# Manta-Network/manta-rs

Measured on AMD Instinct MI355X. Metric: G1 MSM Mscalar/s at 2^20, higher is better.
Workload: dtype u32; 1 GPU; 2^20 BLS12-381 G1 variable-base MSM per GPU, uniform scalars resident in HBM; curve=BLS12-381, log_n=20, window_bits=17, msms_in_flight=3

## Files before the change

manta_rs_amd/csrc/msm_accumulate.h:

```cpp
#pragma once
#include "msm_common.h"

namespace mg {

#ifdef MG_ACC_WAVES
#define MG_ACC_ATTR __attribute__((amdgpu_waves_per_eu(MG_ACC_WAVES, MG_ACC_WAVES)))
#else
#define MG_ACC_ATTR
#endif
template <class F, bool PROBE = false>
__global__ __launch_bounds__(256) MG_ACC_ATTR void accumulate_chunks(const u32 *__restrict__ keys, const u32 *__restrict__ vals,
                                                         u32 M, u32 L, u32 invalid, const u32 *__restrict__ bases,
                                                         u32 astride, u32 *__restrict__ buckets,
                                                         u32 *__restrict__ pkeys, u32 *__restrict__ ppts, u32 T,
                                                         const u32 *__restrict__ count, unsigned long long *__restrict__ clk,
                                                         u32 adapt) {
    const u32 t = blockIdx.x * blockDim.x + threadIdx.x;
    if (t >= T) return;
    long long c0 = 0;
    unsigned long long w0 = 0;
    if constexpr (PROBE)
        if (t == 0) c0 = clock64(), w0 = wall_clock64();
    if (count) {
        M = *count;
        if (adapt) {
            const u32 l = (M + T - 1) / T;
            L = l > L ? l : L;
        }
    }
    const size_t begin = (size_t)t * L;
    size_t end = begin + L;
    if (end > M) end = M;
    u32 cur = begin < M ? keys[begin] : invalid;
    if (cur == invalid) {
        pkeys[2 * t] = invalid;
        pkeys[2 * t + 1] = invalid;
        return;
    }
    XYZZ<F> acc = XYZZ<F>::inf();
    bool first = true;
    for (size_t j = begin; j < end; ++j) {
        const u32 k = keys[j];
        if (k != cur) {
            if (first) {
                pkeys[2 * t] = cur;
                acc.store(ppts + (size_t)(2 * t) * XYZZ<F>::WORDS);
                first = false;
            } else {
                acc.store(buckets + (size_t)cur * XYZZ<F>::WORDS);
            }
            acc = XYZZ<F>::inf();
            cur = k;
            if (k == invalid) break;
        }
        const u32 v = vals[j];
        const Affine<F> p = Affine<F>::load(bases + (size_t)(v & 0x7fffffffu) * astride);
        acc.madd_throughput(p, (v >> 31) != 0);
    }
    if (first) {
        pkeys[2 * t] = cur;
        acc.store(ppts + (size_t)(2 * t) * XYZZ<F>::WORDS);
        pkeys[2 * t + 1] = cur;
        XYZZ<F>::inf().store(ppts + (size_t)(2 * t + 1) * XYZZ<F>::WORDS);
    } else {
        pkeys[2 * t + 1] = cur;
        acc.store(ppts + (size_t)(2 * t + 1) * XYZZ<F>::WORDS);
    }
    if constexpr (PROBE)
        if (t == 0) clk[0] = (unsigned long long)(clock64() - c0), clk[1] = wall_clock64() - w0;
}

template <class F> struct AccSingle {
    static constexpr int XW = XYZZ<F>::WORDS;
    static constexpr int PAIR = F::EXT ? 1 : 0;
    static constexpr int SLOTS = 256 >> PAIR, PER = SLOTS / 64;
    typedef CoopAdd<F, false> Coop;
    static constexpr size_t LDS_BYTES = ((size_t)SLOTS * XW + Coop::LDS_WORDS) * 4;
};
template <class F>
__global__ __launch_bounds__(256) MG_TAIL_ATTR void accumulate_single(const u32 *__restrict__ vals, u32 M, u32 L, const u32 *__restrict__ bases,
                                                                      u32 astride, u32 *__restrict__ pkeys, u32 *__restrict__ ppts, u32 T,
                                                                      const u32 *__restrict__ count, u32 adapt, u32 invalid) {
    extern __shared__ __attribute__((aligned(16))) u32 acc_single_lds[];
    constexpr int XW = AccSingle<F>::XW, PAIR = AccSingle<F>::PAIR, SLOTS = AccSingle<F>::SLOTS, PER = AccSingle<F>::PER;
    u32 *xs = acc_single_lds;
    u32 *cx = acc_single_lds + SLOTS * XW;
    const u32 t = blockIdx.x * blockDim.x + threadIdx.x;
    const int lane = threadIdx.x & 63, wave = threadIdx.x >> 6;
    if (count) {
        M = *count;
        if (adapt) {
            const u32 l = (M + T - 1) / T;
            L = l > L ? l : L;
        }
    }
    XYZZ<F> acc = XYZZ<F>::inf();
    const size_t begin = (size_t)t * L;
    size_t end = begin + L;
    if (end > M) end = M;
    if (t < T)
        for (size_t j = begin; j < end; ++j) {
            const u32 v = vals[j];
            const Affine<F> p = Affine<F>::load(bases + (size_t)(v & 0x7fffffffu) * astride);
            acc.madd_throughput(p, (v >> 31) != 0);
        }
    if ((size_t)blockIdx.x * blockDim.x * L >= M) {
        if (threadIdx.x == 0) pkeys[blockIdx.x] = invalid;
        return;
    }
    if constexpr (PAIR) acc.add(XYZZ<F>::shfl(acc, lane ^ 1));
    if (!PAIR || !(lane & 1)) acc.store(xs + (size_t)(threadIdx.x >> PAIR) * XW);
    __syncthreads();
    acc = XYZZ<F>::load(xs + (size_t)(lane * PER) * XW);
#pragma unroll 1
    for (int k = 1; k < PER; ++k) AccSingle<F>::Coop::add(acc, XYZZ<F>::load(xs + (size_t)(lane * PER + k) * XW), cx, wave, lane);
#pragma unroll 1
    for (int d = 1; d < 64; d <<= 1) AccSingle<F>::Coop::add(acc, XYZZ<F>::shfl(acc, lane ^ d), cx, wave, lane);
    if (threadIdx.x == 0) {
        pkeys[blockIdx.x] = 0u;
        acc.store(ppts + (size_t)blockIdx.x * XW);
    }
}

#ifdef MG_CALIBRATION
template <class F>
__global__ __launch_bounds__(256) void gather_only_chunks(const u32 *__restrict__ keys, const u32 *__restrict__ vals,
                                                          u32 M, u32 L, u32 invalid, const u32 *__restrict__ bases,
                                                          u32 astride, u32 *__restrict__ pkeys, u32 T,
                                                          const u32 *__restrict__ count) {
    const u32 t = blockIdx.x * blockDim.x + threadIdx.x;
    if (t >= T) return;
    if (count) M = *count;
    const size_t begin = (size_t)t * L;
    size_t end = begin + L;
    if (end > M) end = M;
    u32 x = 0;
    for (size_t j = begin; j < end; ++j) {
        const u32 k = keys[j];
        if (k == invalid) break;
        const u32 v = vals[j];
        const uint4 *p = reinterpret_cast<const uint4 *>(bases + (size_t)(v & 0x7fffffffu) * astride);
#pragma unroll
        for (int q = 0; q < (int)(Affine<F>::WORDS + 3) / 4; ++q) {
            const uint4 w = p[q];
            x ^= w.x ^ w.y ^ w.z ^ w.w;
        }
        x ^= k;
    }
    pkeys[2 * t] = invalid;
    pkeys[2 * t + 1] = invalid;
    if (x == 0x9e3779b9u) pkeys[2 * t] = invalid - 1;
}
#endif

}
```

manta_rs_amd/csrc/msm_engine.h:

```cpp
#pragma once
#include "msm_common.h"
#include "msm_digits.h"
#include "msm_accumulate.h"
#include "msm_reduce.h"
#include "msm_tables.h"

namespace mg {

template <class Curve, int GROUP> struct GT;
template <class Curve> struct GT<Curve, 1> {
#ifdef MG_G1_SATURATED
    typedef Fp<typename Curve::Fq> F;
#else
    typedef FpR<typename Curve::Fq> F;
#endif
    typedef Fp<typename Curve::Fq> FIO;
    typedef host::HFp<typename Curve::Fq> HF;
};
template <class Curve> struct GT<Curve, 2> {
#ifdef MG_G2_SATURATED
    typedef Fp2<typename Curve::Fq> F;
#else
    typedef Fp2R<typename Curve::Fq> F;
#endif
// ... 400 lines not shown
            if (hipEventElapsedTime(&ms, ws->t0, ws->t1) == hipSuccess) set_last_accumulate_ms(ms);
            const unsigned long long ck[2] = {((volatile unsigned long long *)ws->h_clk)[0], ((volatile unsigned long long *)ws->h_clk)[1]};
            int khz = 0, dev = 0;
            if (ck[1] && hipGetDevice(&dev) == hipSuccess &&
                hipDeviceGetAttribute(&khz, hipDeviceAttributeWallClockRate, dev) == hipSuccess)
                set_last_accumulate_mhz((float)((double)ck[0] / (double)ck[1] * (double)khz / 1e3));
        }
        const MsmPlan &pl = ws->plan;
        const MsmTail &t = ws->tail;
        const u32 Wb = (u32)pl.Wb, segs = t.segs, T1 = t.T1, nP = t.nP;
        const u32 *st = (const u32 *)ws->h_stage;
        for (u32 q = 0; q < ws->batch; ++q) {
        HP total = HP::inf();
        for (int w = (int)((q + 1) * Wb) - 1; w >= (int)(q * Wb); --w) {
            HP win;
            if (t.kind == TAIL_WINDOW_SUMS) {
                win = HP::from_xyzz_words(st + (size_t)w * XW_IO);
            } else if (t.kind == TAIL_X_SUMS) {
                const HP X = HP::from_xyzz_words(st + ((size_t)w * 2 + 0) * XW_IO);
                const HP sumS = HP::from_xyzz_words(st + ((size_t)w * 2 + 1) * XW_IO);
                win = HP::add(sumS, HP::mul_pow2(X, 6));
            } else {
                const u32 *A1 = st + ((size_t)w * T1) * XW_IO;
                const u32 *S1 = st + ((size_t)segs * T1 + (size_t)w * T1) * XW_IO;
                const u32 *P0 = st + ((size_t)segs * 2 * T1 + (size_t)w * nP) * XW_IO;
                HP sumS = HP::inf(), run = HP::inf(), uA = HP::inf();
                for (int u = (int)T1 - 1; u >= 0; --u) {
                    sumS = HP::add(sumS, HP::from_xyzz_words(S1 + (size_t)u * XW_IO));
                    if (u >= 1) {
                        run = HP::add(run, HP::from_xyzz_words(A1 + (size_t)u * XW_IO));
                        uA = HP::add(uA, run);
                    }
                }
                HP X = HP::add(sumS, HP::mul_pow2(uA, 6));
                HP sumP = HP::inf();
                for (u32 u = 0; u < nP; ++u) sumP = HP::add(sumP, HP::from_xyzz_words(P0 + (size_t)u * XW_IO));
                win = HP::add(sumP, HP::mul_pow2(X, 6));
            }
            if (t.tail_shift) win = HP::mul_pow2(win, t.tail_shift);
            for (u32 e = 0; e < t.n_extra; ++e) {
                const HP x = HP::from_xyzz_words(st + (t.extra_off_pts + (size_t)e * segs + (size_t)w) * XW_IO);
                win = HP::add(win, t.extra_shift[e] ? HP::mul_pow2(x, t.extra_shift[e]) : x);
            }
            if (w != (int)((q + 1) * Wb) - 1) total = HP::mul_pow2(total, (unsigned)pl.c);
            total = HP::add(total, win);
        }
        hp(out + q) = total;
        }
        return MG_OK;
    }

    int msm_fold_device(MsmWorkspace *ws, u32 *d_out, size_t out_stride_words, hipStream_t on = nullptr) override {
        if (!ws || !ws->pending || !d_out || !ws->tail.d_tail) return MG_ERR_STATE;
        const MsmTail &t = ws->tail;
        if (ws->plan.Wb != 1) return MG_ERR_STATE;
        FoldDesc d{t.d_tail, ws->extra.as<u32>(), t.kind, t.T1, t.nP, t.segs, t.n_extra, t.tail_shift, {}};
        for (u32 e = 0; e < t.n_extra; ++e) d.extra_shift[e] = t.extra_shift[e];
        hipLaunchKernelGGL((fold_windows<F>), dim3(ws->batch), dim3(64), 0, on ? on : msm_stream_of(ws), d, d_out, out_stride_words);
        MG_HIP(hipGetLastError());
        return MG_OK;
    }
    int msm_discard(MsmWorkspace *ws) override {
        if (!ws) return MG_ERR_STATE;
        ws->pending = 0;
        MG_HIP(hipStreamSynchronize(msm_stream_of(ws)));
        return MG_OK;
    }

    int fixed_base_mul(const u32 *base_affine_host, const u32 *d_scalars, size_t n, u32 *d_out_affine,
                       hipStream_t s) override {
        if (!s) s = setup_stream();
        u32 *d_base = nullptr, *tmp = nullptr;
        MG_HIP(hipMalloc((void **)&d_base, AW_IO * 4));
        hipError_t e = hipMalloc((void **)&tmp, n * XW_IO * 4);
        if (e != hipSuccess) {
            hipFree(d_base);
            set_last_hip_error(e, "hipMalloc(fixed_base tmp)", __FILE__, __LINE__);
            return MG_ERR_OOM;
        }
        hipMemcpyAsync(d_base, base_affine_host, AW_IO * 4, hipMemcpyHostToDevice, s);
        constexpr int KB = 16;
        u32 *t_xyzz = nullptr, *t_aff = nullptr;
        if (n >= msm_knobs().fixed_base_table_min) {
            constexpr size_t TN = 32 * 255;
            if (hipMalloc((void **)&t_xyzz, TN * XW_IO * 4) == hipSuccess && hipMalloc((void **)&t_aff, TN * AW_IO * 4) == hipSuccess) {
                hipLaunchKernelGGL((fixed_base_table_kernel<FIO>), dim3(cdiv(TN, 256)), dim3(256), 0, s, d_base, t_xyzz);
                hipLaunchKernelGGL((xyzz_to_affine_batch<FIO, KB>), dim3(cdiv(cdiv(TN, KB), 256)), dim3(256), 0, s, t_xyzz, TN, t_aff,
                                   (u32)AW_IO);
                hipLaunchKernelGGL((fixed_base_mul_table_kernel<FIO>), dim3(cdiv(n, 256)), dim3(256), 0, s, t_aff, d_scalars, n, tmp);
            } else {
                (void)hipGetLastError();
                if (t_xyzz) hipFree(t_xyzz);
                t_xyzz = nullptr;
            }
        }
        if (!t_xyzz)
        hipLaunchKernelGGL((fixed_base_mul_kernel<FIO>), dim3(cdiv(n, 256)), dim3(256), 0, s, d_base, d_scalars, n, tmp);
        hipLaunchKernelGGL((xyzz_to_affine_batch<FIO, KB>), dim3(cdiv(cdiv(n, KB), 256)), dim3(256), 0, s, tmp, n,
                           d_out_affine, (u32)AW_IO);
        e = hipStreamSynchronize(s);
        hipFree(d_base);
        hipFree(tmp);
        if (t_xyzz) hipFree(t_xyzz);
        if (t_aff) hipFree(t_aff);
        if (e != hipSuccess) {
            set_last_hip_error(e, "fixed_base_mul", __FILE__, __LINE__);
            return MG_ERR_HIP;
        }
        return MG_OK;
    }

    int ec_elementwise(int op, const u32 *a_host, const u32 *b_host, size_t n, u32 *out_affine_host) override {
        return ec_elementwise_impl(op, a_host, b_host, n, out_affine_host, false);
    }
    int ec_elementwise_xyzz(int op, const u32 *a_host, const u32 *b_host, size_t n, u32 *out_xyzz_host) override {
        return ec_elementwise_impl(op, a_host, b_host, n, out_xyzz_host, true);
    }
    int ec_mul_xyzz_begin(const u32 *a_host, const u32 *k_host, size_t n, MsmWorkspace *ws, const u32 *glv_beta_std) override {
        if (!a_host || !k_host || !n || !ws) return MG_ERR_ARG;
        const size_t ab = n * AW_IO * 4, bb = n * 32 + (glv_beta_std ? (size_t)AW_IO / 2 * 4 : 0), tb = n * XW_IO * 4;
        int rc = ws->scratch.reserve(ab + bb + tb);
        if (rc) return rc;
        unsigned char *d = (unsigned char *)ws->scratch.p;
        hipError_t e = hipMemcpyAsync(d, a_host, ab, hipMemcpyHostToDevice, ws->stream);
        if (e == hipSuccess) e = hipMemcpyAsync(d + ab, k_host, n * 32, hipMemcpyHostToDevice, ws->stream);
        if (e == hipSuccess && glv_beta_std)
            e = hipMemcpyAsync(d + ab + n * 32, glv_beta_std, (size_t)AW_IO / 2 * 4, hipMemcpyHostToDevice, ws->stream);
        if (e == hipSuccess) {
            hipLaunchKernelGGL((ec_elementwise_kernel<F>), dim3(cdiv(n, 256)), dim3(256), 0, ws->stream, glv_beta_std ? 6 : 3, (const u32 *)d,
                               (const u32 *)(d + ab), n, (u32 *)(d + ab + bb));
            e = hipGetLastError();
        }
        if (e != hipSuccess) {
            hipStreamSynchronize(ws->stream);
            set_last_hip_error(e, "ec_mul_xyzz", __FILE__, __LINE__);
            return MG_ERR_HIP;
        }
        return MG_OK;
    }
    const u32 *ec_mul_xyzz_device(MsmWorkspace *ws, size_t n, bool glv) const override {
        const size_t ab = n * AW_IO * 4, bb = n * 32 + (glv ? (size_t)AW_IO / 2 * 4 : 0);
        return ws && ws->scratch.p ? (const u32 *)((unsigned char *)ws->scratch.p + ab + bb) : nullptr;
    }
    int ec_mul_xyzz_finish(MsmWorkspace *ws, size_t n, u32 *out_xyzz_host, bool glv) override {
        if (!ws || !n || !out_xyzz_host) return MG_ERR_ARG;
        const size_t ab = n * AW_IO * 4, bb = n * 32 + (glv ? (size_t)AW_IO / 2 * 4 : 0), tb = n * XW_IO * 4;
        hipError_t e = hipMemcpyAsync(out_xyzz_host, (unsigned char *)ws->scratch.p + ab + bb, tb, hipMemcpyDeviceToHost, ws->stream);
        const hipError_t e2 = hipStreamSynchronize(ws->stream);
        if (e == hipSuccess) e = e2;
        if (e != hipSuccess) {
            set_last_hip_error(e, "ec_mul_xyzz", __FILE__, __LINE__);
            return MG_ERR_HIP;
        }
        return MG_OK;
    }
    void xyzz_batch_to_affine(const u32 *xyzz_host, size_t n, u32 *out_affine_host) const override {
        typedef decltype(HP{}.x) HF;
        std::vector<HF> den(n), pre(n);
        HF acc = HF::one();
        for (size_t i = 0; i < n; ++i) {
            const HP q = HP::from_xyzz_words(xyzz_host + i * XW_IO);
            den[i] = q.is_inf() ? HF::one() : HF::mul(q.zz, q.zzz);
            pre[i] = acc;
            acc = HF::mul(acc, den[i]);
        }
        HF inv = HF::inv(acc);
        for (size_t i = n; i-- > 0;) {
            const HP q = HP::from_xyzz_words(xyzz_host + i * XW_IO);
            const HF t = HF::mul(inv, pre[i]);
            inv = HF::mul(inv, den[i]);
            u32 *o = out_affine_host + i * AW_IO;
            if (q.is_inf()) {
                std::memset(o, 0, AW_IO * 4);
                continue;
            }
            HF::mul(q.x, HF::mul(t, q.zzz)).store_words(o);
            HF::mul(q.y, HF::mul(t, q.zz)).store_words(o + HF::WORDS);
        }
    }
    int ec_elementwise_impl(int op, const u32 *a_host, const u32 *b_host, size_t n, u32 *out_host, bool xyzz) {
        if (op < 0 || op > 5 || !a_host || !out_host || n == 0 || (op != 2 && !b_host)) return MG_ERR_ARG;
        const size_t ab = n * AW_IO * 4, bb = op == 3 ? n * 32 : (op == 5 ? 32 : ab);
        u32 *da = nullptr, *db = nullptr, *tmp = nullptr, *dout = nullptr;
        hipStream_t st = stream_pool_get_normal();
        hipError_t e = st ? hipSuccess : hipErrorOutOfMemory;
        if (e == hipSuccess) e = hipMalloc((void **)&da, ab);
        if (e == hipSuccess) e = hipMalloc((void **)&db, bb);
        if (e == hipSuccess) e = hipMalloc((void **)&tmp, n * XW_IO * 4);
        if (e == hipSuccess && !xyzz) e = hipMalloc((void **)&dout, ab);
        if (e == hipSuccess) e = hipMemcpyAsync(da, a_host, ab, hipMemcpyHostToDevice, st);
        if (e == hipSuccess && op != 2) e = hipMemcpyAsync(db, b_host, bb, hipMemcpyHostToDevice, st);
        if (e == hipSuccess) {
            hipLaunchKernelGGL((ec_elementwise_kernel<F>), dim3(cdiv(n, 256)), dim3(256), 0, st, op, da, db, n, tmp);
            if (xyzz) {
                e = hipMemcpyAsync(out_host, tmp, n * XW_IO * 4, hipMemcpyDeviceToHost, st);
            } else {
                constexpr int KB = 16;
                hipLaunchKernelGGL((xyzz_to_affine_batch<FIO, KB>), dim3(cdiv(cdiv(n, KB), 256)), dim3(256), 0, st, tmp, n, dout,
                                   (u32)AW_IO);
                e = hipMemcpyAsync(out_host, dout, ab, hipMemcpyDeviceToHost, st);
            }
        }
        if (st) {
            const hipError_t e2 = hipStreamSynchronize(st);
            if (e == hipSuccess) e = e2;
            stream_pool_put_normal(st);
        }
        hipFree(da);
        hipFree(db);
        hipFree(tmp);
        if (dout) hipFree(dout);
        if (e != hipSuccess) {
            set_last_hip_error(e, "ec_elementwise", __FILE__, __LINE__);
            return e == hipErrorOutOfMemory ? MG_ERR_OOM : MG_ERR_HIP;
        }
        return MG_OK;
    }

    int group_ntt(const u32 *in_affine_host, unsigned lg, const u32 *d_twiddles_mont, const u32 *n_inv_canonical,
                  u32 *out_affine_host) override {
        if (!in_affine_host || !out_affine_host || lg > 26 || (lg > 0 && !d_twiddles_mont)) return MG_ERR_ARG;
        const size_t n = (size_t)1 << lg, ab = n * AW_IO * 4;
        u32 *d_in = nullptr, *d_pts = nullptr, *d_std = nullptr, *d_out = nullptr, *d_sc = nullptr;
        hipError_t e = hipMalloc((void **)&d_in, ab);
        if (e == hipSuccess) e = hipMalloc((void **)&d_pts, n * XW * 4);
        if (e == hipSuccess) e = hipMalloc((void **)&d_std, n * XW_IO * 4);
        if (e == hipSuccess) e = hipMalloc((void **)&d_out, ab);
        if (e == hipSuccess && n_inv_canonical) e = hipMalloc((void **)&d_sc, 32);
        if (e == hipSuccess) e = memcpy_sync(d_in, in_affine_host, ab, hipMemcpyHostToDevice);
        if (e == hipSuccess && n_inv_canonical) e = memcpy_sync(d_sc, n_inv_canonical, 32, hipMemcpyHostToDevice);
        if (e == hipSuccess) {
            hipLaunchKernelGGL((group_ntt_load_kernel<F>), dim3(cdiv(n, 256)), dim3(256), 0, setup_stream(), d_in, lg, d_pts);
            for (unsigned s = 1; s <= lg; ++s)
                hipLaunchKernelGGL((group_ntt_stage_kernel<F, FrC>), dim3(cdiv(n / 2, 256)), dim3(256), 0, setup_stream(), d_pts, d_twiddles_mont, lg, s);
            hipLaunchKernelGGL((group_scale_store_kernel<F>), dim3(cdiv(n, 256)), dim3(256), 0, setup_stream(), d_pts, (const u32 *)d_sc, n, d_std);
            constexpr int KB = 16;
            hipLaunchKernelGGL((xyzz_to_affine_batch<FIO, KB>), dim3(cdiv(cdiv(n, KB), 256)), dim3(256), 0, setup_stream(), d_std, n, d_out, (u32)AW_IO);
            e = memcpy_sync(out_affine_host, d_out, ab, hipMemcpyDeviceToHost);
        }
        hipFree(d_in), hipFree(d_pts), hipFree(d_std), hipFree(d_out), hipFree(d_sc);
        if (e != hipSuccess) {
            set_last_hip_error(e, "group_ntt", __FILE__, __LINE__);
            return e == hipErrorOutOfMemory ? MG_ERR_OOM : MG_ERR_HIP;
        }
        return MG_OK;
    }

    int sum_affine(const u32 *d_pts, size_t n, HostPoint *out) override {
        const u32 T = n < 4096 ? (u32)(n ? n : 1) : 4096;
        u32 *tmp = nullptr;
        MG_HIP(hipMalloc((void **)&tmp, (size_t)T * XW_IO * 4));
        hipLaunchKernelGGL((sum_affine_kernel<FIO>), dim3(cdiv(T, 256)), dim3(256), 0, setup_stream(), d_pts, n, T, tmp);
        std::vector<u32> h((size_t)T * XW_IO);
        hipError_t e = memcpy_sync(h.data(), tmp, h.size() * 4, hipMemcpyDeviceToHost);
        hipFree(tmp);
        if (e != hipSuccess) {
            set_last_hip_error(e, "sum_affine", __FILE__, __LINE__);
            return MG_ERR_HIP;
        }
        HP acc = HP::inf();
        for (u32 t = 0; t < T; ++t) acc = HP::add(acc, HP::from_xyzz_words(h.data() + (size_t)t * XW_IO));
        hp(out) = acc;
        return MG_OK;
    }

  private:
    struct Launch {
        const BaseSet *bs;
        const u32 *d_scalars;
        MsmWorkspace *ws;
        hipStream_t s, side;
        size_t n, n_scalars, scalar_stride_words;
        int scalar_mode;
        u32 batch, nsets;
        bool batched_pass, sparse;
        MsmPlan pl;
        size_t M;
        int end_bit;
        u32 KB, seg_keys, nb, invalid, T, sort_mask = 0xffffffffu, sort_inv = 0xffffffffu;
        bool direct, per_query, acc_single;
        u32 *d_count;
        const u32 *skeys, *svals;
        u32 parts;
        const u32 *rin;
        u32 rstride, roff, rn;
        MsmTail tail;
    };

    int launch_reserve(Launch &r) {
        MsmWorkspace *const ws = r.ws; const MsmPlan &pl = r.pl;
        const size_t M = r.M = r.n * (size_t)pl.W * r.batch;
        r.KB = pl.full ? 1u : pl.B;
        if (M >= (1ull << 31) || (size_t)r.batch * r.nsets * pl.Wb * r.KB >= (1ull << 24)) return MG_ERR_ARG;
        if (pl.full) r.sparse = true;
        const u32 seg_keys = r.seg_keys = (u32)pl.Wb * r.KB;
        const u32 nb = r.nb = r.batch * r.nsets * seg_keys;
        const u32 invalid = r.invalid = nb;
        int rc;
        if ((rc = ws->keys_in.reserve(M * 4)) || (rc = ws->keys_out.reserve(M * 4)) ||
            (rc = ws->vals_in.reserve(M * 4)) || (rc = ws->vals_out.reserve(M * 4)))
            return rc;
        if ((rc = ws->sort_tmp.reserve(sort_pairs_temp_bytes(M))) || (rc = ws->buckets.reserve((size_t)(nb + 1) * XW * 4))) return rc;
        const u32 T = r.T = cdiv(M, pl.L);
        if ((rc = ws->pkeys[0].reserve((size_t)2 * T * 4)) || (rc = ws->ppts[0].reserve((size_t)2 * T * XW * 4)))
            return rc;
        const u32 waves1 = cdiv((size_t)2 * T, 64);
        if ((rc = ws->pkeys[1].reserve((size_t)2 * waves1 * 4)) ||
            (rc = ws->ppts[1].reserve((size_t)2 * waves1 * XW * 4)))
            return rc;

        if ((size_t)pl.W * r.bs->n * (pl.full ? pl.B : 1u) >= (1ull << 31)) return MG_ERR_ARG;
        int end_bit = 1;
        while ((1u << end_bit) <= invalid) ++end_bit;
        int end_bit_real = 1;
        while (nb > 1 && (1u << end_bit_real) <= nb - 1) ++end_bit_real;
        if ((end_bit + 7) / 8 > (end_bit_real + 7) / 8) r.sparse = true;
        if (r.sparse) end_bit = end_bit_real;
        if (msm_knobs().sort_low && !r.sparse && r.batch > 1 && r.nsets == 1 && (seg_keys & (seg_keys - 1)) == 0) {
            int eb = 1;
            while ((1u << eb) <= seg_keys) ++eb;
            if ((eb + 7) / 8 < (end_bit + 7) / 8) r.sort_mask = seg_keys - 1, r.sort_inv = invalid, end_bit = eb;
        }
        r.end_bit = end_bit;
        if (r.sparse && sort_pairs_takes_device_count(end_bit)) {
            if ((rc = ws->count.reserve(256))) return rc;
            r.d_count = ws->count.as<u32>();
        }
#ifdef MG_NO_DIRECT
        r.direct = false;
#else
        r.direct = nb == 1;
#endif
        if (r.direct && ((rc = ws->redA.reserve((size_t)XWM * 4)) || (rc = ws->redS.reserve((size_t)XWM * 4)))) return rc;
        ws->timed = kernel_timing() && !ws->capturing;
        if (ws->timed && !ws->h_clk) MG_HIP(hipHostMalloc((void **)&ws->h_clk, 64, hipHostMallocDefault));
        return MG_OK;
    }
    static constexpr int XWM = XW > XW_IO ? XW : XW_IO;

    void launch_digits(Launch &r) {
        MsmWorkspace *const ws = r.ws; const MsmPlan &pl = r.pl; const BaseSet *const bs = r.bs; hipStream_t s = r.s;
        ZeroRanges zr{};
        zr.p[0] = r.d_count, zr.n[0] = r.d_count ? 1u : 0u;
        zr.p[1] = r.direct ? ws->redS.as<u32>() : ws->buckets.as<u32>();
        zr.n[1] = r.direct ? (u32)XWM : (u32)((size_t)(r.nb + 1) * XW);
        zr.p[2] = ws->timed ? (u32 *)ws->h_clk : nullptr, zr.n[2] = ws->timed ? 4u : 0u;
        const u32 most = zr.n[1] > 4u ? zr.n[1] : 4u;
        hipLaunchKernelGGL((zero_ranges<F>), dim3(most > 256u * 1024u ? 1024u : cdiv(most, 256)), dim3(256), 0, s, zr);
        const u32 dthreads = r.d_count ? msm_knobs().digits_threads : 256u;
        const u32 nsets = r.nsets;
        r.per_query = pl.full && nsets > 1 && nsets <= BaseSet::MAX_SETS && r.batch == 1 && r.d_count && !msm_knobs().z3_sort &&
                      bs->set_first[nsets] == (u32)bs->n;
        if (r.per_query) {
            for (u32 q = 0; q < nsets; ++q) {
                const u32 lo = bs->set_first[q], hi = bs->set_first[q + 1];
                if (hi <= lo) continue;
                hipLaunchKernelGGL((digits_kernel<FrC>), dim3(cdiv(hi - lo, dthreads), 1), dim3(dthreads), 0, s, r.d_scalars, hi, pl.c,
                                   pl.W, pl.B, 2, (u32)bs->n, r.scalar_mode, r.invalid, ws->keys_in.as<u32>(), ws->vals_in.as<u32>(),
                                   (const u32 *)bs->d_map, (u32)r.n_scalars, r.scalar_stride_words, r.seg_keys, r.d_count, nsets,
                                   (u32)bs->set_len, lo);
            }
        } else
            hipLaunchKernelGGL((digits_kernel<FrC>), dim3(cdiv(r.n, dthreads), r.batch), dim3(dthreads), 0, s, r.d_scalars, (u32)r.n,
                               pl.c, pl.W, pl.B, pl.full ? 2 : (pl.precomp ? 1 : 0), (u32)bs->n, r.scalar_mode, r.invalid,
                               ws->keys_in.as<u32>(), ws->vals_in.as<u32>(), (const u32 *)bs->d_map, (u32)r.n_scalars,
                               r.scalar_stride_words, r.seg_keys, r.d_count, nsets, (u32)bs->set_len);
        r.batch *= nsets;
    }

    int launch_sort(Launch &r) {
        MsmWorkspace *const ws = r.ws;
        const bool no_sort = (r.nb == 1 || r.per_query) && r.d_count;
        r.skeys = no_sort ? ws->keys_in.as<u32>() : ws->keys_out.as<u32>();
        r.svals = no_sort ? ws->vals_in.as<u32>() : ws->vals_out.as<u32>();
        return no_sort ? MG_OK
                       : sort_pairs(ws->keys_in.as<u32>(), ws->keys_out.as<u32>(), ws->vals_in.as<u32>(), ws->vals_out.as<u32>(), r.M,
                                    r.end_bit, ws->sort_tmp.p, sort_pairs_temp_bytes(r.M), r.s, r.d_count, r.sort_mask, r.sort_inv);
    }

    int launch_accumulate(Launch &r) {
        MsmWorkspace *const ws = r.ws; const MsmPlan &pl = r.pl; const BaseSet *const bs = r.bs; hipStream_t s = r.s;
        u32 Tl = r.T, adapt = 0;
        u32 Lk = pl.L;
        const bool acc_single_on = ((msm_knobs().acc_single >> (GROUP - 1)) & 1) != 0;
        const int dev_now = current_device();
        const bool acc_single = r.acc_single = r.nb == 1 && r.d_count && acc_single_on && !(kernel_timing() && !ws->capturing) &&
                                               dev_now >= 0 && dev_now < 64 && occ_[dev_now].cus.load(std::memory_order_acquire) &&
                                               occ_[dev_now].blocks_single;
        if (r.d_count) {
            const u32 tgt = acc_round_lanes(r.batched_pass, acc_single);
            if (tgt && Tl > tgt) Tl = tgt, adapt = 1;
            else if (tgt && !r.batched_pass && pl.L > 6) adapt = 1;
            if (adapt && Lk > 6) Lk = 6;
        }
        const u32 M = (u32)r.M, invalid = r.invalid;
        if (ws->timed) MG_HIP(hipEventRecord(ws->t0, s));
#ifdef MG_CALIBRATION
        static const bool gather_only = std::getenv("MANTA_ACC_GATHER_ONLY") != nullptr;
        if (gather_only)
            hipLaunchKernelGGL((gather_only_chunks<F>), dim3(cdiv(r.T, 256)), dim3(256), 0, s, ws->keys_out.as<u32>(),
                               ws->vals_out.as<u32>(), M, pl.L, invalid, bs->d_pts, (u32)AWS, ws->pkeys[0].as<u32>(), r.T,
                               (const u32 *)r.d_count);
        else
#endif
        if (acc_single)
            hipLaunchKernelGGL((accumulate_single<F>), dim3(cdiv(Tl, 256)), dim3(256), AccSingle<F>::LDS_BYTES, s, r.svals, M, Lk, bs->d_pts, (u32)AWS,
                               ws->pkeys[0].as<u32>(), ws->ppts[0].as<u32>(), Tl, (const u32 *)r.d_count, adapt, invalid);
        else
        if (ws->timed)
            hipLaunchKernelGGL((accumulate_chunks<F, true>), dim3(cdiv(Tl, 256)), dim3(256), 0, s, r.skeys,
                               r.svals, M, Lk, invalid, bs->d_pts, (u32)AWS, ws->buckets.as<u32>(),
                               ws->pkeys[0].as<u32>(), ws->ppts[0].as<u32>(), Tl, (const u32 *)r.d_count, ws->h_clk, adapt);
        else
            hipLaunchKernelGGL((accumulate_chunks<F, false>), dim3(cdiv(Tl, 256)), dim3(256), 0, s, r.skeys,
                               r.svals, M, Lk, invalid, bs->d_pts, (u32)AWS, ws->buckets.as<u32>(),
                               ws->pkeys[0].as<u32>(), ws->ppts[0].as<u32>(), Tl, (const u32 *)r.d_count, (unsigned long long *)nullptr, adapt);
        if (ws->timed) MG_HIP(hipEventRecord(ws->t1, s));
        r.parts = acc_single ? cdiv(Tl, 256) : 2 * Tl;
        return MG_OK;
    }

    void launch_merge(Launch &r) {
        MsmWorkspace *const ws = r.ws;
        u32 *const std_final = r.direct ? ws->redS.as<u32>() : (u32 *)nullptr;
        u32 cnt = r.parts;
        int src = 0;
        for (int level = 0;; ++level) {
            u32 G = level == 0 && !r.acc_single ? merge_g1(r.M) : 2;
            if (cnt <= 512) G = cnt <= 64 ? 1 : cdiv(cnt, 64);
            const u32 waves = cdiv(cdiv(cnt, G), 64);
            const int fin = waves == 1;
            merge_partials_launch(r.s, waves, ws->pkeys[src].as<u32>(), ws->ppts[src].as<u32>(), cnt, G, r.invalid, fin,
                                  ws->buckets.as<u32>(), ws->pkeys[1 - src].as<u32>(), ws->ppts[1 - src].as<u32>(), std_final);
            if (fin) break;
            cnt = 2 * waves;
            src ^= 1;
        }
    }

    int launch_front_levels(Launch &r) {
        MsmWorkspace *const ws = r.ws; const MsmPlan &pl = r.pl; hipStream_t s = r.s; MsmTail &t = r.tail;
        const u32 segs = t.segs = r.batch * (u32)pl.Wb;
        r.rin = ws->buckets.as<u32>(), r.rstride = r.KB, r.roff = 0, r.rn = r.KB;
        const MsmKnobs &rk = msm_knobs();
        const int lgS_eff = rk.lgS >= 0 ? rk.lgS : 3;
        const u32 min_items = r.batched_pass ? rk.min_items_batch : rk.min_items;
        if (lgS_eff <= 0 || r.rn < min_items) return MG_OK;
        hipStreamCaptureStatus cst = hipStreamCaptureStatusNone;
        const bool being_captured = hipStreamIsCapturing(s, &cst) != hipSuccess || cst != hipStreamCaptureStatusNone;
        if (!ws->capturing && !ws->run_on && !ws->in_graph_slot && !being_captured && rk.side) {
            if (!(r.side = engine_side_stream())) return MG_ERR_HIP;
            if (!ws->side_fork) {
                MG_HIP(hipEventCreateWithFlags(&ws->side_fork, hipEventDisableTiming));
                MG_HIP(hipEventCreateWithFlags(&ws->side_join, hipEventDisableTiming));
            }
            ws->side_stream = r.side;
        }
        for (int pass = 0; pass < 2; ++pass) {
            size_t used = 0;
            auto take = [&](size_t pts) {
                u32 *p = pass ? ws->front.as<u32>() + used * XW : nullptr;
                used += pts;
                return p;
            };
            const u32 *in = ws->buckets.as<u32>();
            u32 stride = pl.B, off = 0, n = pl.B, shift = 0, ne = 0;
            while (n >= min_items && ne < (u32)MsmTail::MAX_EXTRA) {
                const int lg = (size_t)segs * n >= ((size_t)1 << 18) ? rk.lgS0 : (rk.lgS < 0 && n >= (1u << 16) ? 4 : lgS_eff);
                const u32 lanes = cdiv(n, 1u << lg);
                u32 *A = take((size_t)segs * lanes), *Sx = take((size_t)segs * lanes);
                if (pass) serial_reduce_launch(s, (size_t)segs * lanes, in, stride, off, n, 1u << lg, lanes, A, Sx);
                hipStream_t ps = r.side ? r.side : s;
                if (pass && r.side) {
                    MG_HIP(hipEventRecord(ws->side_fork, s));
                    MG_HIP(hipStreamWaitEvent(r.side, ws->side_fork, 0));
                }
                const u32 *pin = Sx;
                u32 pcnt = lanes;
                while (pcnt > 64) {
                    int plg = rk.lgSP;
                    while (plg > 1 && (pcnt >> plg) < 32 && pcnt > 64u << 1) --plg;
                    const u32 pl2 = cdiv(pcnt, 1u << plg);
                    u32 *tp = take((size_t)segs * pl2);
                    if (pass) serial_reduce_launch(ps, (size_t)segs * pl2, pin, pcnt, 0u, pcnt, 1u << plg, pl2, tp, (u32 *)nullptr);
                    pin = tp;
                    pcnt = pl2;
                }
                if (pass)
                    tile_reduce_launch(ps, segs, true, pin, pcnt, 0u, pcnt, 1u, ws->extra.as<u32>() + (size_t)ne * segs * XW_IO,
                                       (u32 *)nullptr, 1);
                t.extra_shift[ne++] = shift;
                shift += lg;
                in = A, stride = lanes, off = 1, n = lanes - 1;
            }
            int rc;
            if (pass) r.rin = in, r.rstride = stride, r.roff = off, r.rn = n, t.tail_shift = shift, t.n_extra = ne;
            else if ((rc = ws->front.reserve(used * XW * 4)) || (rc = ws->extra.reserve((size_t)MsmTail::MAX_EXTRA * segs * XW_IO * 4)))
                return rc;
        }
        return MG_OK;
    }

    int launch_scan_tail(Launch &r) {
        MsmWorkspace *const ws = r.ws; hipStream_t s = r.s; MsmTail &t = r.tail;
        const u32 segs = t.segs, T0 = cdiv(r.rn, 64);
        int rc;
        if (r.direct) {
            t.extra_off_pts = segs;
        } else if (T0 == 1) {
            if ((rc = ws->redA.reserve((size_t)segs * XWM * 4)) || (rc = ws->redS.reserve((size_t)segs * XWM * 4))) return rc;
            tile_reduce_launch(s, segs, r.rn > 1, r.rin, r.rstride, r.roff, r.rn, 1u, ws->redA.as<u32>(), ws->redS.as<u32>(), 1);
            t.extra_off_pts = segs;
        } else if (T0 <= 64) {
            if ((rc = ws->redA.reserve((size_t)segs * T0 * XW * 4)) || (rc = ws->redS.reserve((size_t)segs * T0 * XW * 4)) ||
                (rc = ws->misc.reserve((size_t)segs * 2 * XW_IO * 4)))
                return rc;
            tile_reduce_launch(s, segs * T0, true, r.rin, r.rstride, r.roff, r.rn, T0, ws->redA.as<u32>(), ws->redS.as<u32>(), 0);
            reduce_level1_launch(s, segs, ws->redA.as<u32>(), ws->redS.as<u32>(), T0, ws->misc.as<u32>());
            t.kind = TAIL_X_SUMS;
            t.extra_off_pts = (size_t)segs * 2;
        } else {
            if ((rc = ws->redA.reserve((size_t)segs * T0 * XWM * 4)) || (rc = ws->redS.reserve((size_t)segs * T0 * XWM * 4)))
                return rc;
            tile_reduce_launch(s, segs * T0, false, r.rin, r.rstride, r.roff, r.rn, T0, ws->redA.as<u32>(), ws->redS.as<u32>(), 0);
            const u32 T1 = t.T1 = cdiv(T0 - 1, 64);
            const u32 nP = t.nP = cdiv(T0, 64);
            if ((rc = ws->misc.reserve((size_t)segs * (2 * T1 + nP) * XW_IO * 4))) return rc;
            u32 *A1 = ws->misc.as<u32>();
            u32 *S1 = A1 + (size_t)segs * T1 * XW_IO;
            u32 *P0 = S1 + (size_t)segs * T1 * XW_IO;
            tile_reduce_launch(s, segs * T1, true, ws->redA.as<u32>(), T0, 1u, T0 - 1, T1, A1, S1, 1);
            tile_reduce_launch(s, segs * nP, true, ws->redS.as<u32>(), T0, 0u, T0, nP, P0, (u32 *)nullptr, 1);
            t.kind = TAIL_TWO_LEVELS;
            t.extra_off_pts = (size_t)segs * (2 * T1 + nP);
        }
        t.d_tail = t.kind == TAIL_WINDOW_SUMS ? ws->redS.as<u32>() : ws->misc.as<u32>();
        return MG_OK;
    }

    int launch_stage(Launch &r) {
        MsmWorkspace *const ws = r.ws; hipStream_t s = r.s; MsmTail &t = r.tail;
        const size_t stage_pts = t.extra_off_pts, extra_pts = (size_t)t.n_extra * t.segs;
        const bool own_stage = ws->notify || (stage_pts + extra_pts) * XW_IO <= 16384;
        if (const int rc = stage_reserve(ws, (stage_pts + extra_pts) * XW_IO * 4)) return rc;
        if (!own_stage) MG_HIP(hipMemcpyAsync(ws->h_stage, t.d_tail, stage_pts * XW_IO * 4, hipMemcpyDeviceToHost, s));
        if (t.n_extra && r.side) {
            MG_HIP(hipEventRecord(ws->side_join, r.side));
            MG_HIP(hipStreamWaitEvent(s, ws->side_join, 0));
        }
        if (t.n_extra && !own_stage)
            MG_HIP(hipMemcpyAsync((u32 *)ws->h_stage + stage_pts * XW_IO, ws->extra.p, extra_pts * XW_IO * 4, hipMemcpyDeviceToHost, s));
        if (own_stage) {
            if (ws->notify && !ws->h_flag) {
                MG_HIP(hipHostMalloc((void **)&ws->h_flag, 64, hipHostMallocDefault));
                *ws->h_flag = 0;
            }
            hipLaunchKernelGGL(stage_and_notify_kernel, dim3(1), dim3(256), 0, s, t.d_tail, (u32 *)ws->h_stage, (u32)(stage_pts * XW_IO),
                               (const u32 *)ws->extra.p, (u32 *)ws->h_stage + stage_pts * XW_IO, (u32)(extra_pts * XW_IO),
                               ws->notify ? ws->h_flag : (u32 *)nullptr);
        }
        return MG_OK;
    }
};

}
```

manta_rs_amd/csrc/msm_reduce.h:

```cpp
#pragma once
#include "msm_common.h"

namespace mg {

template <class F, bool COOP> struct TailAdd;
template <class F> struct TailAdd<F, false> {
    static constexpr bool UNIFORM = false;
    const int lane = threadIdx.x & 63;
    MG_DEV u32 unit() const { return blockIdx.x * (blockDim.x >> 6) + (threadIdx.x >> 6); }
    MG_DEV bool writer() const { return true; }
    MG_DEV void add_if(XYZZ<F> &acc, const XYZZ<F> &o, bool take) const {
        if (take) acc.add(o);
    }
    MG_DEV void publish() const {}
};
template <class F> struct TailAdd<F, true> {
    static constexpr bool UNIFORM = true;
    u32 *lds;
    const int lane = threadIdx.x & 63, pw = threadIdx.x >> 6;
    MG_DEV u32 unit() const { return blockIdx.x; }
    MG_DEV bool writer() const { return pw == 0; }
    MG_DEV void add_if(XYZZ<F> &acc, XYZZ<F> o, bool take) const {
        if (!take) o = XYZZ<F>::inf();
        CoopAdd<F>::add(acc, o, lds, pw, lane);
    }
    MG_DEV void publish() const {
        __threadfence_block();
        __syncthreads();
    }
};

template <class F, class A>
MG_DEV void merge_body(const A a, u32 *__restrict__ pkeys, u32 *__restrict__ ppts, u32 cnt, u32 G, u32 invalid, int final_level,
                       u32 *__restrict__ buckets, u32 *__restrict__ okeys, u32 *__restrict__ opts, u32 *__restrict__ std_final) {
    constexpr size_t XW = XYZZ<F>::WORDS;
    const u32 wave = a.unit();
    const int lane = a.lane;
    const size_t b = ((size_t)wave * 64 + lane) * G;
    u32 kh = invalid, cur = invalid;
    bool single = true, open = false;
    XYZZ<F> acc = XYZZ<F>::inf();
    if (b < cnt) {
        cur = pkeys[b];
        if (cur != invalid) {
            kh = cur;
            acc = XYZZ<F>::load(ppts + b * XW);
            open = true;
        }
    }
    if constexpr (A::UNIFORM) {
        for (u32 off = 1; off < G; ++off) {
            const size_t j = b + off;
            const bool have = open && j < cnt;
            const u32 k = have ? pkeys[j] : invalid;
            XYZZ<F> p = XYZZ<F>::inf();
            if (have && k != invalid) p = XYZZ<F>::load(ppts + j * XW);
            const bool same = have && k == cur;
            if (have && k != cur) {
                if (a.writer()) acc.store(single ? ppts + b * XW : buckets + (size_t)cur * XW);
                single = false;
                cur = k;
                acc = p;
                if (k == invalid) open = false;
            }
            if (__any(same && !p.is_inf())) a.add_if(acc, p, same);
        }
    } else if (open) {
        const size_t end = b + G < cnt ? b + G : cnt;
        for (size_t j = b + 1; j < end; ++j) {
            const u32 k = pkeys[j];
            if (k != cur) {
                if (single) {
                    acc.store(ppts + b * XW);
                    single = false;
                } else {
                    acc.store(buckets + (size_t)cur * XW);
                }
                cur = k;
                acc = XYZZ<F>::inf();
                if (k == invalid) break;
                acc = XYZZ<F>::load(ppts + j * XW);
            } else {
                const XYZZ<F> p = XYZZ<F>::load(ppts + j * XW);
                if (!p.is_inf()) acc.add(p);
            }
        }
    }
    const u32 kt = cur;
    a.publish();
    for (int d = 1; d < 64; d <<= 1) {
        const u32 nk = __shfl_up(kt, d, 64);
        const bool take = (lane >= d) && (nk == kt) && (kt != invalid);
        if (!__any(take)) break;
        a.add_if(acc, XYZZ<F>::shfl(acc, lane - d < 0 ? lane : lane - d), take);
    }
    const u32 prev_kt = __shfl_up(kt, 1, 64), next_kh = __shfl_down(kh, 1, 64);
    const u32 key0 = __shfl(kh, 0, 64);
    const bool need_in = !single && lane > 0 && prev_kt == kh;
    const bool any_in = __any(need_in);
    XYZZ<F> prev = XYZZ<F>::inf();
    if (any_in) prev = XYZZ<F>::shfl(acc, lane > 0 ? lane - 1 : 0);
    const bool cont = lane < 63 && next_kh == kt;
    if (a.writer() && kt != invalid && !cont) {
        if (final_level) {
            if (std_final) acc.store_std(std_final + (size_t)kt * XYZZ<typename F::Std>::WORDS);
            else acc.store(buckets + (size_t)kt * XW);
        } else if (kt == key0) {
            okeys[2 * wave] = kt;
            acc.store(opts + (size_t)(2 * wave) * XW);
            if (lane == 63) {
                okeys[2 * wave + 1] = kt;
                XYZZ<F>::inf().store(opts + (size_t)(2 * wave + 1) * XW);
            }
        } else if (lane == 63) {
            okeys[2 * wave + 1] = kt;
            acc.store(opts + (size_t)(2 * wave + 1) * XW);
        } else {
            acc.store(buckets + (size_t)kt * XW);
        }
    }
    if (a.writer() && !final_level && lane == 63 && kt == invalid) {
        okeys[2 * wave + 1] = invalid;
        if (key0 == invalid) okeys[2 * wave] = invalid;
    }
    XYZZ<F> h = XYZZ<F>::inf();
    if (!single) h = XYZZ<F>::load(ppts + b * XW);
    if (any_in) a.add_if(h, prev, need_in);
    if (a.writer() && !single) {
        if (!final_level && kh == key0) {
            okeys[2 * wave] = kh;
            h.store(opts + (size_t)(2 * wave) * XW);
        } else if (final_level && std_final) {
            h.store_std(std_final + (size_t)kh * XYZZ<typename F::Std>::WORDS);
        } else {
            h.store(buckets + (size_t)kh * XW);
        }
    }
}
template <class F>
__global__ __launch_bounds__(256) MG_TAIL_ATTR void merge_partials(u32 *__restrict__ pkeys, u32 *__restrict__ ppts, u32 cnt, u32 G,
                                                      u32 invalid, int final_level, u32 *__restrict__ buckets,
                                                      u32 *__restrict__ okeys, u32 *__restrict__ opts, u32 n_waves,
                                                      u32 *__restrict__ std_final) {
    MG_PRIO_FOR(F);
    const TailAdd<F, false> a{};
    if (a.unit() >= n_waves) return;
    merge_body<F>(a, pkeys, ppts, cnt, G, invalid, final_level, buckets, okeys, opts, std_final);
}
template <class F>
__global__ __launch_bounds__(256) MG_TAIL_COOP_ATTR void merge_partials_coop(u32 *__restrict__ pkeys, u32 *__restrict__ ppts, u32 cnt, u32 G,
                                                           u32 invalid, int final_level, u32 *__restrict__ buckets,
                                                           u32 *__restrict__ okeys, u32 *__restrict__ opts,
                                                           u32 *__restrict__ std_final) {
    MG_PRIO_FOR(F);
    __shared__ __attribute__((aligned(16))) u32 lds[CoopAdd<F>::LDS_WORDS];
    merge_body<F>(TailAdd<F, true>{lds}, pkeys, ppts, cnt, G, invalid, final_level, buckets, okeys, opts, std_final);
}

template <class F, class A>
MG_DEV void tile_reduce_body(const A a, const u32 *__restrict__ in, u32 seg_stride , u32 item_off, u32 n_items,
                             u32 tiles_per_seg, u32 *__restrict__ outA, u32 *__restrict__ outS, int std_out) {
    const u32 wave = a.unit();
    const int lane = a.lane;
    const u32 seg = wave / tiles_per_seg, tile = wave % tiles_per_seg;
    const u32 idx = tile * 64 + lane;
    XYZZ<F> acc = XYZZ<F>::inf();
    if (idx < n_items) acc = XYZZ<F>::load(in + ((size_t)seg * seg_stride + item_off + idx) * XYZZ<F>::WORDS);
    int top = 1;
    {
        const u32 left = n_items - tile * 64;
        const int lim = left < 64 ? (int)left : 64;
        while (top < lim) top <<= 1;
    }
    for (int d = 1; d < top; d <<= 1)
        a.add_if(acc, XYZZ<F>::shfl(acc, lane + d > 63 ? lane : lane + d), lane + d < 64);
    constexpr int SW = XYZZ<typename F::Std>::WORDS;
    const bool store = a.writer() && lane == 0;
    if (store) {
        if (std_out)
            acc.store_std(outA + (size_t)wave * SW);
        else
            acc.store(outA + (size_t)wave * XYZZ<F>::WORDS);
    }
    if (outS) {
        for (int d = top >> 1; d >= 1; d >>= 1)
            a.add_if(acc, XYZZ<F>::shfl(acc, lane + d > 63 ? lane : lane + d), lane < d);
        if (store) {
            if (std_out)
                acc.store_std(outS + (size_t)wave * SW);
            else
                acc.store(outS + (size_t)wave * XYZZ<F>::WORDS);
        }
    }
}
template <class F>
__global__ __launch_bounds__(256) MG_TAIL_ATTR void tile_reduce(const u32 *__restrict__ in, u32 seg_stride ,
                                                   u32 item_off, u32 n_items, u32 tiles_per_seg, u32 n_waves,
                                                   u32 *__restrict__ outA, u32 *__restrict__ outS, int std_out) {
    MG_PRIO_FOR(F);
    const TailAdd<F, false> a{};
    if (a.unit() >= n_waves) return;
    tile_reduce_body<F>(a, in, seg_stride, item_off, n_items, tiles_per_seg, outA, outS, std_out);
}
template <class F>
__global__ __launch_bounds__(256) MG_TAIL_COOP_ATTR void tile_reduce_coop(const u32 *__restrict__ in, u32 seg_stride ,
                                                        u32 item_off, u32 n_items, u32 tiles_per_seg,
                                                        u32 *__restrict__ outA, u32 *__restrict__ outS, int std_out) {
    MG_PRIO_FOR(F);
    __shared__ __attribute__((aligned(16))) u32 lds[CoopAdd<F>::LDS_WORDS];
    tile_reduce_body<F>(TailAdd<F, true>{lds}, in, seg_stride, item_off, n_items, tiles_per_seg, outA, outS, std_out);
}

template <class F, class A>
MG_DEV void serial_reduce_body(const A a, const u32 *__restrict__ in, u32 seg_stride , u32 item_off, u32 n_items, u32 S,
                               u32 lanes_per_seg, u32 n_lanes, u32 *__restrict__ outA, u32 *__restrict__ outS) {
    constexpr size_t XW = XYZZ<F>::WORDS;
    const u32 g = a.unit() * 64 + a.lane;
    const bool live = g < n_lanes;
    if (!A::UNIFORM && !live) return;
    const u32 seg = live ? g / lanes_per_seg : 0, l = live ? g % lanes_per_seg : 0;
    const u32 i0 = l * S;
    const u32 *base = in + ((size_t)seg * seg_stride + item_off) * XW;
    XYZZ<F> acc = XYZZ<F>::inf(), sum = XYZZ<F>::inf();
    if constexpr (A::UNIFORM) {
        for (u32 j = S; j-- > 0;) {
            const u32 i = i0 + j;
            const bool have = live && i < n_items;
            XYZZ<F> x = XYZZ<F>::inf();
            if (have) x = XYZZ<F>::load(base + (size_t)i * XW);
            a.add_if(acc, x, have);
            if (outS) a.add_if(sum, acc, have);
        }
    } else {
        const u32 i1 = i0 + S < n_items ? i0 + S : n_items;
        for (u32 i = i1; i-- > i0;) {
            acc.add(XYZZ<F>::load(base + (size_t)i * XW));
            if (outS) sum.add(acc);
        }
    }
    if (live && a.writer()) {
        acc.store(outA + (size_t)g * XW);
        if (outS) sum.store(outS + (size_t)g * XW);
    }
}
template <class F>
__global__ __launch_bounds__(256) MG_SERIAL_ATTR void serial_reduce(const u32 *__restrict__ in, u32 seg_stride , u32 item_off,
                                                     u32 n_items, u32 S, u32 lanes_per_seg, u32 n_lanes,
                                                     u32 *__restrict__ outA, u32 *__restrict__ outS) {
    MG_PRIO_FOR(F);
    serial_reduce_body<F>(TailAdd<F, false>{}, in, seg_stride, item_off, n_items, S, lanes_per_seg, n_lanes, outA, outS);
}
template <class F>
__global__ __launch_bounds__(256) MG_TAIL_COOP_ATTR void serial_reduce_coop(const u32 *__restrict__ in, u32 seg_stride , u32 item_off,
                                                          u32 n_items, u32 S, u32 lanes_per_seg, u32 n_lanes,
                                                          u32 *__restrict__ outA, u32 *__restrict__ outS) {
    MG_PRIO_FOR(F);
    __shared__ __attribute__((aligned(16))) u32 lds[CoopAdd<F>::LDS_WORDS];
    serial_reduce_body<F>(TailAdd<F, true>{lds}, in, seg_stride, item_off, n_items, S, lanes_per_seg, n_lanes, outA, outS);
}

template <class F, class A>
MG_DEV void reduce_level1_body(const A a, u32 seg, int part, const u32 *__restrict__ A0, const u32 *__restrict__ S0, u32 T0,
                               u32 *__restrict__ out_std) {
    constexpr int XW = XYZZ<F>::WORDS;
    constexpr int SW = XYZZ<typename F::Std>::WORDS;
    const int lane = a.lane;
    int top = 1;
    while (top < (int)T0) top <<= 1;
    XYZZ<F> acc = XYZZ<F>::inf();
    if (part == 0) {
        if (lane >= 1 && lane < (int)T0) acc = XYZZ<F>::load(A0 + ((size_t)seg * T0 + lane) * XW);
        for (int d = 1; d < top; d <<= 1)
            a.add_if(acc, XYZZ<F>::shfl(acc, lane + d > 63 ? lane : lane + d), lane + d < 64);
        if (lane == 0) acc = XYZZ<F>::inf();
    } else {
        if (lane < (int)T0) acc = XYZZ<F>::load(S0 + ((size_t)seg * T0 + lane) * XW);
    }
    for (int d = top >> 1; d >= 1; d >>= 1)
        a.add_if(acc, XYZZ<F>::shfl(acc, lane + d > 63 ? lane : lane + d), lane < d);
    if (a.writer() && lane == 0) acc.store_std(out_std + ((size_t)seg * 2 + part) * SW);
}
template <class F>
__global__ __launch_bounds__(128) MG_TAIL_ATTR void reduce_level1(const u32 *__restrict__ A0, const u32 *__restrict__ S0, u32 T0,
                                                     u32 *__restrict__ out_std) {
    MG_PRIO_FOR(F);
    reduce_level1_body<F>(TailAdd<F, false>{}, blockIdx.x, threadIdx.x >> 6, A0, S0, T0, out_std);
}
template <class F>
__global__ __launch_bounds__(256) MG_TAIL_COOP_ATTR void reduce_level1_coop(const u32 *__restrict__ A0, const u32 *__restrict__ S0, u32 T0,
                                                          u32 *__restrict__ out_std) {
    MG_PRIO_FOR(F);
    __shared__ __attribute__((aligned(16))) u32 lds[CoopAdd<F>::LDS_WORDS];
    reduce_level1_body<F>(TailAdd<F, true>{lds}, blockIdx.x >> 1, blockIdx.x & 1, A0, S0, T0, out_std);
}

struct FoldDesc {
    const u32 *tail, *extra;
    u32 kind, T1, nP, segs, n_extra, tail_shift;
    u32 extra_shift[8];
};
static_assert(sizeof(FoldDesc::extra_shift) == sizeof(MsmTail::extra_shift), "FoldDesc::extra_shift holds MsmTail::MAX_EXTRA shifts");
template <class F>
__global__ __launch_bounds__(64) void fold_windows(FoldDesc d, u32 *__restrict__ out, size_t out_stride) {
    MG_PRIO_FOR(F);
    typedef typename F::Std S;
    constexpr int SW = XYZZ<S>::WORDS;
    const u32 q = blockIdx.x;
    auto ld = [](const u32 *p) {
        const XYZZ<S> s = XYZZ<S>::load(p);
        if (s.is_inf()) return XYZZ<F>::inf();
        return XYZZ<F>{F::from_std(s.x), F::from_std(s.y), F::from_std(s.zz), F::from_std(s.zzz)};
    };
    auto pow2 = [](XYZZ<F> p, u32 k) {
        for (u32 i = 0; i < k; ++i) p = XYZZ<F>::dbl(p);
        return p;
    };
    XYZZ<F> win = XYZZ<F>::inf();
    if (d.kind == TAIL_WINDOW_SUMS) {
        win = ld(d.tail + (size_t)q * SW);
    } else if (d.kind == TAIL_X_SUMS) {
        win = pow2(ld(d.tail + ((size_t)q * 2 + 0) * SW), 6);
        win.add(ld(d.tail + ((size_t)q * 2 + 1) * SW));
    } else {
        const u32 *A1 = d.tail + (size_t)q * d.T1 * SW;
        const u32 *S1 = d.tail + ((size_t)d.segs * d.T1 + (size_t)q * d.T1) * SW;
        const u32 *P0 = d.tail + ((size_t)d.segs * 2 * d.T1 + (size_t)q * d.nP) * SW;
        XYZZ<F> sumS = XYZZ<F>::inf(), run = XYZZ<F>::inf(), uA = XYZZ<F>::inf();
        for (int u = (int)d.T1 - 1; u >= 0; --u) {
            sumS.add(ld(S1 + (size_t)u * SW));
            if (u >= 1) {
                run.add(ld(A1 + (size_t)u * SW));
                uA.add(run);
            }
        }
        XYZZ<F> X = pow2(uA, 6);
        X.add(sumS);
        win = pow2(X, 6);
        for (u32 u = 0; u < d.nP; ++u) win.add(ld(P0 + (size_t)u * SW));
    }
    if (d.tail_shift) win = pow2(win, d.tail_shift);
    for (u32 e = 0; e < d.n_extra; ++e) win.add(pow2(ld(d.extra + ((size_t)e * d.segs + q) * SW), d.extra_shift[e]));
    if (threadIdx.x == 0) win.store_std(out + (size_t)q * out_stride);
}

}
```

Measured before the change: 408.3 Mscalar/s.

## Fuse workgroup-level partial merge into accumulate_chunks for G1

Measured after the change: 356.8 Mscalar/s. 0.874x the previous value.

```diff
diff --git a/manta_rs_amd/csrc/msm_accumulate.h b/manta_rs_amd/csrc/msm_accumulate.h
--- a/manta_rs_amd/csrc/msm_accumulate.h
+++ b/manta_rs_amd/csrc/msm_accumulate.h
@@ -1,5 +1,6 @@
 #pragma once
 #include "msm_common.h"
+#include "msm_reduce.h"
 
 namespace mg {
 
@@ -8,6 +9,11 @@
 #else
 #define MG_ACC_ATTR
 #endif
+template <class F> struct AccMerge {
+    static constexpr bool ON = !F::EXT;
+    static constexpr int PARK_WORDS = ON ? 256 * XYZZ<F>::WORDS : 4, EDGE_WORDS = ON ? 8 * XYZZ<F>::WORDS : 4;
+    static MG_HD u32 parts(u32 lanes) { return ON ? 2 * ((lanes + 255) / 256) : 2 * lanes; }
+};
 template <class F, bool PROBE = false>
 __global__ __launch_bounds__(256) MG_ACC_ATTR void accumulate_chunks(const u32 *__restrict__ keys, const u32 *__restrict__ vals,
                                                          u32 M, u32 L, u32 invalid, const u32 *__restrict__ bases,
@@ -15,8 +21,14 @@
                                                          u32 *__restrict__ pkeys, u32 *__restrict__ ppts, u32 T,
                                                          const u32 *__restrict__ count, unsigned long long *__restrict__ clk,
                                                          u32 adapt) {
+    constexpr bool WG = AccMerge<F>::ON;
+    constexpr int XW = XYZZ<F>::WORDS;
+    __shared__ __attribute__((aligned(16))) u32 park[AccMerge<F>::PARK_WORDS];
+    __shared__ __attribute__((aligned(16))) u32 wpts[AccMerge<F>::EDGE_WORDS];
+    __shared__ u32 wkeys[8];
     const u32 t = blockIdx.x * blockDim.x + threadIdx.x;
-    if (t >= T) return;
+    if constexpr (!WG)
+        if (t >= T) return;
     long long c0 = 0;
     unsigned long long w0 = 0;
     if constexpr (PROBE)
@@ -31,33 +43,53 @@
     const size_t begin = (size_t)t * L;
     size_t end = begin + L;
     if (end > M) end = M;
-    u32 cur = begin < M ? keys[begin] : invalid;
-    if (cur == invalid) {
-        pkeys[2 * t] = invalid;
-        pkeys[2 * t + 1] = invalid;
-        return;
-    }
+    u32 cur = t < T && begin < M ? keys[begin] : invalid;
+    if constexpr (!WG)
+        if (cur == invalid) {
+            pkeys[2 * t] = invalid;
+            pkeys[2 * t + 1] = invalid;
+            return;
+        }
+    const u32 kh = cur;
     XYZZ<F> acc = XYZZ<F>::inf();
     bool first = true;
-    for (size_t j = begin; j < end; ++j) {
-        const u32 k = keys[j];
-        if (k != cur) {
-            if (first) {
-                pkeys[2 * t] = cur;
-                acc.store(ppts + (size_t)(2 * t) * XYZZ<F>::WORDS);
+    if (cur != invalid)
+        for (size_t j = begin; j < end; ++j) {
+            const u32 k = keys[j];
+            if (k != cur) {
+                if (!first) {
+                    acc.store(buckets + (size_t)cur * XW);
+                } else if constexpr (WG) {
+                    acc.store(park + threadIdx.x * XW);
+                } else {
+                    pkeys[2 * t] = cur;
+                    acc.store(ppts + (size_t)(2 * t) * XW);
+                }
                 first = false;
-            } else {
-                acc.store(buckets + (size_t)cur * XYZZ<F>::WORDS);
+                acc = XYZZ<F>::inf();
+                cur = k;
+                if (k == invalid) break;
             }
+            const u32 v = vals[j];
+            const Affine<F> p = Affine<F>::load(bases + (size_t)(v & 0x7fffffffu) * astride);
+            acc.madd_throughput(p, (v >> 31) != 0);
+        }
+    if constexpr (WG) {
+        const TailAdd<F, false> a{};
+        const u32 wave = threadIdx.x >> 6;
+        merge_runs<F>(a, 63, kh, cur, first, acc, park + threadIdx.x * XW, invalid, 0, buckets, wkeys, wpts, wave, (u32 *)nullptr);
+        __syncthreads();
+        if (wave == 0) {
+            const u32 l = a.lane < 4 ? a.lane : 0;
+            u32 k0 = invalid, k1 = invalid;
             acc = XYZZ<F>::inf();
-            cur = k;
-            if (k == invalid) break;
+            if (a.lane < 4) {
+                k0 = wkeys[2 * l], k1 = wkeys[2 * l + 1];
+                if (k1 != invalid) acc = XYZZ<F>::load(wpts + (2 * l + (k0 == k1 ? 0 : 1)) * XW);
+            }
+            merge_runs<F>(a, 3, k0, k1, k0 == k1, acc, wpts + 2 * l * XW, invalid, 0, buckets, pkeys, ppts, blockIdx.x, (u32 *)nullptr);
         }
-        const u32 v = vals[j];
-        const Affine<F> p = Affine<F>::load(bases + (size_t)(v & 0x7fffffffu) * astride);
-        acc.madd_throughput(p, (v >> 31) != 0);
-    }
-    if (first) {
+    } else if (first) {
         pkeys[2 * t] = cur;
         acc.store(ppts + (size_t)(2 * t) * XYZZ<F>::WORDS);
         pkeys[2 * t + 1] = cur;
diff --git a/manta_rs_amd/csrc/msm_engine.h b/manta_rs_amd/csrc/msm_engine.h
--- a/manta_rs_amd/csrc/msm_engine.h
+++ b/manta_rs_amd/csrc/msm_engine.h
@@ -726,9 +726,14 @@
             return rc;
         if ((rc = ws->sort_tmp.reserve(sort_pairs_temp_bytes(M))) || (rc = ws->buckets.reserve((size_t)(nb + 1) * XW * 4))) return rc;
         const u32 T = r.T = cdiv(M, pl.L);
-        if ((rc = ws->pkeys[0].reserve((size_t)2 * T * 4)) || (rc = ws->ppts[0].reserve((size_t)2 * T * XW * 4)))
+#ifdef MG_CALIBRATION
+        const size_t parts = (size_t)2 * T;
+#else
+        const size_t parts = AccMerge<F>::parts(T);
+#endif
+        if ((rc = ws->pkeys[0].reserve(parts * 4)) || (rc = ws->ppts[0].reserve(parts * XW * 4)))
             return rc;
-        const u32 waves1 = cdiv((size_t)2 * T, 64);
+        const u32 waves1 = cdiv(parts, 64);
         if ((rc = ws->pkeys[1].reserve((size_t)2 * waves1 * 4)) ||
             (rc = ws->ppts[1].reserve((size_t)2 * waves1 * XW * 4)))
             return rc;
@@ -840,7 +845,10 @@
                                r.svals, M, Lk, invalid, bs->d_pts, (u32)AWS, ws->buckets.as<u32>(),
                                ws->pkeys[0].as<u32>(), ws->ppts[0].as<u32>(), Tl, (const u32 *)r.d_count, (unsigned long long *)nullptr, adapt);
         if (ws->timed) MG_HIP(hipEventRecord(ws->t1, s));
-        r.parts = acc_single ? cdiv(Tl, 256) : 2 * Tl;
+        r.parts = acc_single ? cdiv(Tl, 256) : AccMerge<F>::parts(Tl);
+#ifdef MG_CALIBRATION
+        if (gather_only) r.parts = 2 * r.T;
+#endif
         return MG_OK;
     }
 
@@ -850,7 +858,7 @@
         u32 cnt = r.parts;
         int src = 0;
         for (int level = 0;; ++level) {
-            u32 G = level == 0 && !r.acc_single ? merge_g1(r.M) : 2;
+            u32 G = level == 0 && !r.acc_single && !AccMerge<F>::ON ? merge_g1(r.M) : 2;
             if (cnt <= 512) G = cnt <= 64 ? 1 : cdiv(cnt, 64);
             const u32 waves = cdiv(cdiv(cnt, G), 64);
             const int fin = waves == 1;
diff --git a/manta_rs_amd/csrc/msm_reduce.h b/manta_rs_amd/csrc/msm_reduce.h
--- a/manta_rs_amd/csrc/msm_reduce.h
+++ b/manta_rs_amd/csrc/msm_reduce.h
@@ -30,6 +30,9 @@
     }
 };
 
+template <class F, class A>
+MG_DEV void merge_runs(const A a, int last, u32 kh, u32 kt, bool single, XYZZ<F> &acc, const u32 *head, u32 invalid, int final_level,
+                       u32 *__restrict__ buckets, u32 *okeys, u32 *opts, u32 wave, u32 *__restrict__ std_final);
 template <class F, class A>
 MG_DEV void merge_body(const A a, u32 *__restrict__ pkeys, u32 *__restrict__ ppts, u32 cnt, u32 G, u32 invalid, int final_level,
                        u32 *__restrict__ buckets, u32 *__restrict__ okeys, u32 *__restrict__ opts, u32 *__restrict__ std_final) {
@@ -86,9 +89,15 @@
             }
         }
     }
-    const u32 kt = cur;
     a.publish();
-    for (int d = 1; d < 64; d <<= 1) {
+    merge_runs<F>(a, 63, kh, cur, single, acc, ppts + b * XW, invalid, final_level, buckets, okeys, opts, wave, std_final);
+}
+template <class F, class A>
+MG_DEV void merge_runs(const A a, const int last, const u32 kh, const u32 kt, const bool single, XYZZ<F> &acc, const u32 *head, u32 invalid,
+                       int final_level, u32 *__restrict__ buckets, u32 *okeys, u32 *opts, const u32 wave, u32 *__restrict__ std_final) {
+    constexpr size_t XW = XYZZ<F>::WORDS;
+    const int lane = a.lane;
+    for (int d = 1; d <= last; d <<= 1) {
         const u32 nk = __shfl_up(kt, d, 64);
         const bool take = (lane >= d) && (nk == kt) && (kt != invalid);
         if (!__any(take)) break;
@@ -100,7 +109,7 @@
     const bool any_in = __any(need_in);
     XYZZ<F> prev = XYZZ<F>::inf();
     if (any_in) prev = XYZZ<F>::shfl(acc, lane > 0 ? lane - 1 : 0);
-    const bool cont = lane < 63 && next_kh == kt;
+    const bool cont = lane < last && next_kh == kt;
     if (a.writer() && kt != invalid && !cont) {
         if (final_level) {
             if (std_final) acc.store_std(std_final + (size_t)kt * XYZZ<typename F::Std>::WORDS);
@@ -108,23 +117,23 @@
         } else if (kt == key0) {
             okeys[2 * wave] = kt;
             acc.store(opts + (size_t)(2 * wave) * XW);
-            if (lane == 63) {
+            if (lane == last) {
                 okeys[2 * wave + 1] = kt;
                 XYZZ<F>::inf().store(opts + (size_t)(2 * wave + 1) * XW);
             }
-        } else if (lane == 63) {
+        } else if (lane == last) {
             okeys[2 * wave + 1] = kt;
             acc.store(opts + (size_t)(2 * wave + 1) * XW);
         } else {
             acc.store(buckets + (size_t)kt * XW);
         }
     }
-    if (a.writer() && !final_level && lane == 63 && kt == invalid) {
+    if (a.writer() && !final_level && lane == last && kt == invalid) {
         okeys[2 * wave + 1] = invalid;
         if (key0 == invalid) okeys[2 * wave] = invalid;
     }
     XYZZ<F> h = XYZZ<F>::inf();
-    if (!single) h = XYZZ<F>::load(ppts + b * XW);
+    if (!single) h = XYZZ<F>::load(head);
     if (any_in) a.add_if(h, prev, need_in);
     if (a.writer() && !single) {
         if (!final_level && kh == key0) {
```
